# rknightion/iq-to-audio

Measured on AMD Instinct MI355X. Metric: complex IQ MS/s end-to-end (ingest->48 kHz audio), higher is better.
Workload: dtype i8; 1 GPU; BASELINE config 2: synthetic 60 s @ 10 MS/s int16 I/Q, 1 NFM channel, +25 kHz, bw 12.5 kHz, D=104, 6401 taps, chunk 4194304; frames_per_gpu=600000000, parallelism=1 independent capture(s), one per GPU; RCCL gather of 48 kHz audio only, audio_samples_48k=2879996, mix_sign=1, settle_steps=55

## Files before the change

### include/iqa_hotpath.h

```cpp
#ifndef IQA_HOTPATH_H
#define IQA_HOTPATH_H

#include <stdint.h>

#ifdef __cplusplus
extern "C" {
#endif

#define IQA_ABI_VERSION 1
#define IQA_SUMSQ_SLOTS 8

typedef enum {
    IQA_OK = 0,
    IQA_EINVAL = 1,
    IQA_EHIP = 2,
    IQA_ESTATE = 3
} iqa_status;

typedef enum { IQA_FMT_S16 = 0, IQA_FMT_U8 = 1, IQA_FMT_F32 = 2 } iqa_fmt;

typedef enum { IQA_ORDER_IQ = 0, IQA_ORDER_QI = 1, IQA_ORDER_IQ_INV = 2, IQA_ORDER_QI_INV = 3 } iqa_iq_order;

typedef enum { IQA_DEMOD_NFM = 0, IQA_DEMOD_AM = 1, IQA_DEMOD_USB = 2, IQA_DEMOD_LSB = 3 } iqa_demod;

// ... 39 lines not shown
                        const void *raw_dev, int64_t n_frames, int64_t consumed, int64_t m_first, int64_t n_out,
                        void *z_out_dev, void *stream);

typedef struct {
    const void *afrag_dev;
    void *z_out_dev;
    const void *partial_in_dev;
    void *partial_out_dev;
    double unit, c_re, c_im;
    uint64_t rot_step, rot_base;
    float out_scale_re, out_scale_im;
    int32_t q_group, finalize, conj_sum, rotate;
    int32_t raw_partials;
    int32_t reserved;
} iqa_mfma_lane;
int iqa_channelize_mfma_multi(int32_t fmt, int32_t decimation, int32_t k_first, int32_t k_count,
                              int32_t outputs_per_block, const iqa_mfma_lane *lanes, int32_t n_lanes,
                              const void *raw_dev, int64_t n_frames, int64_t consumed, int64_t m_first,
                              int64_t n_out, void *stream);

int iqa_channelize_mfma_pairs(int32_t fmt, int32_t decimation, int32_t k_first, int32_t k_count,
                              int32_t outputs_per_block, const iqa_mfma_lane *lanes, int32_t n_lanes,
                              const void *raw_dev, int64_t n_frames, int64_t consumed, int64_t m_first,
                              int64_t n_out, void *stream);
int32_t iqa_mfma_ring_pairs(int32_t fmt, int32_t decimation, int32_t k_first, int32_t k_count);
int32_t iqa_mfma_ring_lanes(int32_t fmt, int32_t decimation, int32_t k_first, int32_t k_count, int32_t acc32);
int iqa_mfma_combine(const iqa_chan_params *p, const void *const *partials_dev, int32_t n_partials,
                     const double *raw_scale, int64_t m_first, int64_t n_out, void *z_out_dev, void *stream);

int iqa_history_update(int32_t fmt, int32_t ntaps, const void *hist_dev, const void *raw_dev, int64_t n_frames,
                       void *hist_next_dev, void *stream);


int iqa_oscillator_mix(int32_t fmt, int32_t iq_order, const void *in_dev, int64_t n, double phase0, double step,
                       void *out_dev, void *stream);

int iqa_decimate(const void *in_dev, int64_t n, int64_t first, int32_t D, void *out_dev, int64_t n_out,
                 void *stream);

int iqa_mean_power(const void *z_dev, int64_t n, int64_t skip, void *power_dev, void *stream);

int iqa_mean_power_batch(const void *z_dev, int64_t n_each, int32_t parts, int64_t skip, void *power_dev, void *stream);

int iqa_raw_level(int32_t fmt, const void *raw_dev, int64_t n_values, void *mean_square_out, void *stream);


int iqa_quadrature(const void *z_dev, int64_t n, void *prev_dev, void *out_dev, void *stream);

int iqa_envelope(const void *z_dev, int64_t n, void *out_dev, void *stream);

int iqa_real_part(const void *z_dev, int64_t n, void *out_dev, void *stream);

int64_t iqa_scan_workspace_bytes(int64_t n);
int iqa_deemphasis(const void *x_dev, int64_t n, double alpha, void *state_dev, void *y_dev, void *work_dev,
                   void *stream);
int iqa_dc_block(const void *x_dev, int64_t n, double radius, void *state_dev, void *y_dev, void *work_dev,
                 void *stream);
int iqa_agc(const void *x_dev, int64_t n, double target, double decay, const void *reset_starts_dev,
            int64_t n_resets, void *y_dev, void *work_dev, void *stream);

typedef struct {
    int32_t mode;
    int32_t agc_enabled;
    double deemph_alpha;
    double dc_radius;
    double agc_target;
    double agc_decay;
} iqa_demod_params;
int iqa_demodulate(const iqa_demod_params *p, const void *z_dev, int64_t n, void *state_dev,
                   const void *seg_starts_dev, int64_t n_segs, void *peak_dev, void *sumsq_dev, void *audio_out_dev,
                   void *scratch_dev, void *work_dev, void *stream);
int iqa_demodulate_from_reset(const iqa_demod_params *p, const void *z_dev, int64_t n, void *state_dev,
                              const void *seg_starts_dev, int64_t n_segs, void *peak_dev, void *sumsq_dev,
                              void *audio_out_dev, void *scratch_dev, void *work_dev, void *stream);

int iqa_writer_clip(const void *a_dev, int64_t n, void *peak_dev, const void *seg_starts_dev, int64_t n_segs,
                    void *sumsq_dev, void *out_dev, void *stream);

int iqa_resample(const void *x_dev, int64_t n_in, const void *table_dev, int32_t up, int32_t down, int32_t T,
                 int64_t j0, int64_t n_out, void *y_dev, void *pcm16_dev, void *stream);

int iqa_float_to_pcm16(const void *y_dev, int64_t n, void *pcm_dev, void *stream);


#define IQA_WFM_MAX_TAPS 2047
int64_t iqa_wfm_partials(int64_t n);
int iqa_wfm_stereo(int32_t ntaps, const void *taps_dev, float m_scale, const void *theta_dev, int64_t n, const void *hist_dev,
                   void *m_out_dev, void *a_out_dev, void *b_out_dev, void *partials_dev, void *stream);
int iqa_wfm_matrix(const void *a_dev, const void *b_dev, int64_t n, void *left_dev, void *right_dev, void *stream);


#define IQA_RDS_MAX_HALF 2400
#define IQA_RDS_MAX_DECIM 80
int64_t iqa_rds_hist_len(int32_t ntaps, int32_t half_taps);
int64_t iqa_rds_outputs(int64_t pos, int64_t n, int32_t decim);
int64_t iqa_rds_lds_bytes(int32_t ntaps, int32_t half_taps, int32_t decim);
int iqa_rds_baseband(int32_t ntaps, const void *pilot_taps_dev, int32_t half_taps, const void *mf_taps_dev, int32_t decim,
                     float m_scale, double f_mix, double clock_step, const void *theta_dev, int64_t n, int64_t pos,
                     const void *hist_dev, void *y_out_dev, void *q_out_dev, void *stream);
int64_t iqa_rds_clock_chunks(int64_t n);
int iqa_rds_clock(const void *q_dev, int64_t n, int64_t j_first, double clock_step, void *total_dev, void *work_dev,
                  void *phi_out_dev, void *psi_out_dev, void *stream);
int64_t iqa_rds_timing_partials(int64_t n);
int iqa_rds_timing(const void *y_dev, const void *psi_dev, int64_t n, int64_t j0, void *partials_dev, void *out_dev, void *stream);
int iqa_rds_symbols(const void *y_dev, const void *psi_dev, int64_t n, int64_t j0, double tau, int64_t k_first, int64_t nsym,
                    void *sym_out_dev, void *bits_out_dev, void *stream);
int iqa_rds_syndromes(const void *bits_dev, int64_t nbits, void *words_out_dev, void *synd_out_dev, void *stream);


#define IQA_POCSAG_MAX_SPS 384
#define IQA_POCSAG_BAUDS 3
#define IQA_POCSAG_OFFSETS 545
int iqa_pocsag_integrate(const void *theta_dev, int64_t n, const void *hist_dev, int32_t hist_len,
                         const int32_t window[IQA_POCSAG_BAUDS], void *t_out_dev, void *const s_out_dev[IQA_POCSAG_BAUDS],
                         void *stream);
int iqa_pocsag_sync(const void *s_dev, int64_t n, const int32_t offsets[32], int32_t half_bit, void *score_dev,
                    void *list_dev, int64_t capacity, void *count_dev, void *stream);
int iqa_pocsag_codewords(const void *s_dev, int64_t n, const void *list_dev, int64_t nsync, const void *offsets_dev,
                         void *fixed_out_dev, void *raw_out_dev, void *status_out_dev, void *stream);


#define IQA_AFSK_MAX_SPS 400
#define IQA_AFSK_PHASES 8
#define IQA_AFSK_GAINS 3
#define IQA_AFSK_SLOT_BYTES 332
int iqa_afsk_correlate(const void *theta_dev, int64_t n, const void *hist_dev, int32_t window, const void *taps_dev,
                       void *t_out_dev, void *sign_out_dev, void *e1200_out_dev, void *e2200_out_dev, void *stream);
// ... 113 lines not shown
```

### iq-to-audio_amd/_native.py

```python
from __future__ import annotations

import ctypes
import subprocess
from ctypes import c_double, c_float, c_int32, c_int64, c_uint64, c_void_p
from pathlib import Path

import os

PKG_DIR = Path(__file__).resolve().parent
LIB_PATH = Path(os.environ["IQA_LIB"]).resolve() if os.environ.get("IQA_LIB") else PKG_DIR / "libiqa_hotpath.so"
CSRC_DIR = PKG_DIR / "csrc"

IQA_OK, IQA_EINVAL, IQA_EHIP, IQA_ESTATE = 0, 1, 2, 3
FMT_S16, FMT_U8, FMT_F32 = 0, 1, 2
ORDER = {"iq": 0, "qi": 1, "iq_inv": 2, "qi_inv": 3}
ABI_VERSION = 1


class ChanParams(ctypes.Structure):

    _fields_ = [
        ("fmt", c_int32),
        ("ntaps", c_int32),
        ("decimation", c_int32),
# ... 33 lines not shown
    _fields_ = [("method", c_int32), ("auto_floor", c_int32), ("trim", c_int32), ("out_pcm16", c_int32),
                ("margin_db", c_double), ("transient_margin_db", c_double)]


class SquelchSeg(ctypes.Structure):

    _fields_ = [("n", c_int64), ("in_off", c_int64), ("base", c_int64), ("channels", c_int32), ("window", c_int32),
                ("short_window", c_int32), ("long_window", c_int32), ("hold", c_int32), ("fade", c_int32),
                ("lead", c_int32), ("trail", c_int32), ("manual_floor_db", c_double), ("q_index", c_int64 * 6),
                ("q_gamma", c_float * 3), ("reserved", c_int32)]


class SquelchResult(ctypes.Structure):

    _fields_ = [("noise_floor_db", c_double), ("threshold_db", c_double), ("start", c_int64), ("stop", c_int64)]


SQ_TILE = 2048
SQ_METHOD = {"adaptive": 0, "static": 1, "transient": 2}
SQ_STAGE = {"envelope_db": 0, "level": 1, "threshold": 2, "mask": 3, "dilated": 4, "gain": 5}

DEMOD_MODE = {"nfm": 0, "fm": 0, "am": 1, "usb": 2, "ssb": 2, "lsb": 3}

_SIGNATURES = {
    "iqa_abi_version": (ctypes.c_int, []),
    "iqa_last_error": (ctypes.c_char_p, []),
    "iqa_taps_padded_len": (c_int64, [c_int32]),
    "iqa_channelize": (ctypes.c_int, [ctypes.POINTER(ChanParams), c_void_p, c_void_p, c_int64, c_int64, c_void_p,
                                      c_int64, c_int64, c_void_p, c_void_p]),
    "iqa_mfma_afrag_bytes": (c_int64, [c_int32]),
    "iqa_mfma_ring_bytes": (c_int64, [c_int32]),
    "iqa_mfma_ring_lds_bytes": (c_int64, [c_int32, c_int32, c_int32, c_int32, c_int32]),
    "iqa_mfma_ring_mode": (c_int32, [c_int32, c_int32, c_int32, c_int32, c_int32]),
    "iqa_channelize_mfma": (ctypes.c_int, [ctypes.POINTER(ChanParams), ctypes.POINTER(MfmaParams), c_void_p, c_void_p,
                                           c_int64, c_int64, c_int64, c_int64, c_void_p, c_void_p]),
    "iqa_channelize_mfma_multi": (ctypes.c_int, [c_int32, c_int32, c_int32, c_int32, c_int32, ctypes.POINTER(MfmaLane), c_int32,
                                                 c_void_p, c_int64, c_int64, c_int64, c_int64, c_void_p]),
    "iqa_channelize_mfma_pairs": (ctypes.c_int, [c_int32, c_int32, c_int32, c_int32, c_int32, ctypes.POINTER(MfmaLane), c_int32,
                                                 c_void_p, c_int64, c_int64, c_int64, c_int64, c_void_p]),
    "iqa_mfma_ring_pairs": (c_int32, [c_int32, c_int32, c_int32, c_int32]),
    "iqa_mfma_ring_lanes": (c_int32, [c_int32, c_int32, c_int32, c_int32, c_int32]),
    "iqa_mfma_combine": (ctypes.c_int, [ctypes.POINTER(ChanParams), ctypes.POINTER(c_void_p), c_int32, ctypes.POINTER(c_double),
                                        c_int64, c_int64, c_void_p, c_void_p]),
    "iqa_history_update": (ctypes.c_int, [c_int32, c_int32, c_void_p, c_void_p, c_int64, c_void_p, c_void_p]),
    "iqa_oscillator_mix": (ctypes.c_int, [c_int32, c_int32, c_void_p, c_int64, c_double, c_double, c_void_p, c_void_p]),
    "iqa_decimate": (ctypes.c_int, [c_void_p, c_int64, c_int64, c_int32, c_void_p, c_int64, c_void_p]),
    "iqa_mean_power": (ctypes.c_int, [c_void_p, c_int64, c_int64, c_void_p, c_void_p]),
    "iqa_mean_power_batch": (ctypes.c_int, [c_void_p, c_int64, c_int32, c_int64, c_void_p, c_void_p]),
    "iqa_raw_level": (ctypes.c_int, [c_int32, c_void_p, c_int64, c_void_p, c_void_p]),
    "iqa_quadrature": (ctypes.c_int, [c_void_p, c_int64, c_void_p, c_void_p, c_void_p]),
    "iqa_envelope": (ctypes.c_int, [c_void_p, c_int64, c_void_p, c_void_p]),
    "iqa_real_part": (ctypes.c_int, [c_void_p, c_int64, c_void_p, c_void_p]),
    "iqa_scan_workspace_bytes": (c_int64, [c_int64]),
    "iqa_deemphasis": (ctypes.c_int, [c_void_p, c_int64, c_double, c_void_p, c_void_p, c_void_p, c_void_p]),
    "iqa_dc_block": (ctypes.c_int, [c_void_p, c_int64, c_double, c_void_p, c_void_p, c_void_p, c_void_p]),
    "iqa_agc": (ctypes.c_int, [c_void_p, c_int64, c_double, c_double, c_void_p, c_int64, c_void_p, c_void_p, c_void_p]),
    "iqa_demodulate": (ctypes.c_int, [ctypes.POINTER(DemodParams), c_void_p, c_int64, c_void_p, c_void_p, c_int64, c_void_p,
                                      c_void_p, c_void_p, c_void_p, c_void_p, c_void_p]),
    "iqa_demodulate_from_reset": (ctypes.c_int, [ctypes.POINTER(DemodParams), c_void_p, c_int64, c_void_p, c_void_p, c_int64, c_void_p,
                                      c_void_p, c_void_p, c_void_p, c_void_p, c_void_p]),
    "iqa_writer_clip": (ctypes.c_int, [c_void_p, c_int64, c_void_p, c_void_p, c_int64, c_void_p, c_void_p, c_void_p]),
    "iqa_resample": (ctypes.c_int, [c_void_p, c_int64, c_void_p, c_int32, c_int32, c_int32, c_int64, c_int64, c_void_p,
                                    c_void_p, c_void_p]),
    "iqa_float_to_pcm16": (ctypes.c_int, [c_void_p, c_int64, c_void_p, c_void_p]),
    "iqa_trickle_copy": (ctypes.c_int, [c_void_p, c_void_p, c_int64, c_int32, c_void_p]),
    "iqa_f32_to_s16_exact": (ctypes.c_int, [c_void_p, c_int64, c_void_p, c_void_p, c_void_p]),
    "iqa_f32_split_s16": (ctypes.c_int, [c_void_p, c_int64, c_int32, c_void_p, c_void_p, c_void_p, c_void_p]),
    "iqa_psd_frames": (ctypes.c_int, [c_int32, c_int32, c_void_p, c_int64, c_int64, c_int64, c_int32, c_int32, c_int32, c_void_p,
                                      c_double, c_void_p, c_void_p, c_void_p, c_void_p, c_void_p]),
    "iqa_pair_average_rows": (ctypes.c_int, [c_void_p, c_int32, c_int32, c_void_p, c_void_p]),
    "iqa_wfm_partials": (c_int64, [c_int64]),
    "iqa_wfm_stereo": (ctypes.c_int, [c_int32, c_void_p, c_float, c_void_p, c_int64, c_void_p, c_void_p, c_void_p, c_void_p,
                                      c_void_p, c_void_p]),
    "iqa_wfm_matrix": (ctypes.c_int, [c_void_p, c_void_p, c_int64, c_void_p, c_void_p, c_void_p]),
    "iqa_rds_hist_len": (c_int64, [c_int32, c_int32]),
    "iqa_rds_outputs": (c_int64, [c_int64, c_int64, c_int32]),
    "iqa_rds_lds_bytes": (c_int64, [c_int32, c_int32, c_int32]),
    "iqa_rds_baseband": (ctypes.c_int, [c_int32, c_void_p, c_int32, c_void_p, c_int32, c_float, c_double, c_double, c_void_p,
                                        c_int64, c_int64, c_void_p, c_void_p, c_void_p, c_void_p]),
    "iqa_rds_clock_chunks": (c_int64, [c_int64]),
    "iqa_rds_clock": (ctypes.c_int, [c_void_p, c_int64, c_int64, c_double, c_void_p, c_void_p, c_void_p, c_void_p, c_void_p]),
    "iqa_rds_timing_partials": (c_int64, [c_int64]),
    "iqa_rds_timing": (ctypes.c_int, [c_void_p, c_void_p, c_int64, c_int64, c_void_p, c_void_p, c_void_p]),
    "iqa_rds_symbols": (ctypes.c_int, [c_void_p, c_void_p, c_int64, c_int64, c_double, c_int64, c_int64, c_void_p, c_void_p,
                                       c_void_p]),
    "iqa_rds_syndromes": (ctypes.c_int, [c_void_p, c_int64, c_void_p, c_void_p, c_void_p]),
    "iqa_pocsag_integrate": (ctypes.c_int, [c_void_p, c_int64, c_void_p, c_int32, ctypes.POINTER(c_int32), c_void_p,
                                            ctypes.POINTER(c_void_p), c_void_p]),
    "iqa_pocsag_sync": (ctypes.c_int, [c_void_p, c_int64, ctypes.POINTER(c_int32), c_int32, c_void_p, c_void_p, c_int64, c_void_p,
                                       c_void_p]),
    "iqa_pocsag_codewords": (ctypes.c_int, [c_void_p, c_int64, c_void_p, c_int64, c_void_p, c_void_p, c_void_p, c_void_p, c_void_p]),
    "iqa_afsk_correlate": (ctypes.c_int, [c_void_p, c_int64, c_void_p, c_int32, c_void_p, c_void_p, c_void_p, c_void_p, c_void_p, c_void_p]),
    "iqa_afsk_bits": (ctypes.c_int, [c_void_p, c_int64, c_int32, c_double, c_int64, c_void_p, c_void_p]),
    "iqa_afsk_frames": (ctypes.c_int, [c_void_p, c_int64, ctypes.POINTER(c_int64), c_int32, c_double, c_void_p, c_void_p, c_int64,
                                       c_void_p, c_void_p]),
    "iqa_tones_decimate": (ctypes.c_int, [c_void_p, c_int64, c_int64, c_void_p, c_int32, c_void_p, c_void_p, c_void_p]),
    "iqa_tones_bank": (ctypes.c_int, [c_void_p, c_int64, c_int32, c_int32, c_int32, c_void_p, c_void_p, c_void_p, c_void_p]),
    "iqa_tones_decide": (ctypes.c_int, [c_void_p, c_int64, c_void_p, c_void_p, c_int64, c_int32, c_void_p, c_void_p, c_void_p]),
    "iqa_acars_max": (ctypes.c_int, [c_void_p, c_int64, c_void_p, c_void_p]),
    "iqa_acars_detect": (ctypes.c_int, [c_void_p, c_int64, c_int32, c_int32, c_int32, c_void_p, c_int32, c_int32, c_void_p, c_void_p, c_void_p,
                                        c_void_p, c_void_p, c_void_p]),
    "iqa_acars_bits": (ctypes.c_int, [c_void_p, c_int64, c_int32, c_double, c_int64, c_void_p, c_void_p]),
    "iqa_acars_frames": (ctypes.c_int, [c_void_p, c_int64, ctypes.POINTER(c_int64), c_int32, c_double, c_void_p, c_void_p, c_int64,
                                        c_void_p, c_void_p]),
    "iqa_ais_filter": (ctypes.c_int, [c_void_p, c_int64, c_void_p, c_int32, c_void_p, c_void_p, c_void_p, c_void_p]),
    "iqa_ais_symbols": (ctypes.c_int, [c_void_p, c_int64, c_int32, c_double, c_int64, c_void_p, c_void_p]),
    "iqa_ais_frames": (ctypes.c_int, [c_void_p, c_int64, ctypes.POINTER(c_int64), c_int32, c_double, c_void_p, c_void_p, c_int64,
                                      c_void_p, c_void_p]),
    "iqa_adsb_quantise": (ctypes.c_int, [c_void_p, c_int64, c_void_p, c_void_p]),
    "iqa_adsb_search": (ctypes.c_int, [c_void_p, c_int64, c_void_p, ctypes.POINTER(c_int32), c_int32, c_int32, c_void_p, c_void_p, c_void_p,
                                       c_int64, c_void_p, c_void_p]),
    "iqa_squelch_workspace_bytes": (c_int64, [c_int64, c_int32]),
    "iqa_squelch_stage_offset": (c_int64, [c_int64, c_int32, c_int32]),
# ... 85 lines not shown
```

### iq-to-audio_amd/batch.py

```python
from __future__ import annotations

from ctypes import c_int32, c_int64, c_void_p

import numpy as np

from . import _dev as D
from . import _native as N
from . import dsp_plan as P
from .processing import (PRECISION_GUARD, ChannelBank, ChannelDemod, Channelizer, MixSignProbe, Resampler48k, _ChannelKernel,
                         base_precision, immutable_taps, pick_precision, probe_targets, reserve_pinned_scalars)


def reject_wfm(modes) -> None:
    if any((m or "").lower() == "wfm" for m in modes):
        raise ValueError("wfm targets are not supported by the resident batch runners or sharded runs: "
                         "use ProcessingPipeline / MultiChannelPipeline")


def reject_pocsag(pocsag) -> None:
    if pocsag:
        raise ValueError("pocsag=True is not supported by the resident batch runners or sharded runs: "
                         "use ProcessingPipeline / MultiChannelPipeline")


# ... 58 lines not shown
        self.override = mix_sign_override if mix_sign_override in (1, -1) else None
        self.base_precision = precision or base_precision(demod_mode, agc_enabled)
        self.guard = PRECISION_GUARD if precision_guard is None else float(precision_guard)
        self._guarded = bool(self.guard) and self.override is None and (demod_mode or "").lower() in ("nfm", "fm")
        self._spec_sign, self._spec_precision = 1, self.base_precision
        self.redone = dict(sign=0, precision=0)
        self.n_dec = -(-self.n_frames // self.d)
        self.starts = P.chunk_output_starts(self.chunk, self.d, 0, self.n_frames)
        self.rs = Resampler48k(self.fs_ch)
        self.n48 = self.rs.plan.n_out(self.n_dec)
        self.compute = torch.cuda.current_stream()
        self._compute_raw = int(self.compute.cuda_stream)
        self.aux = D.side_stream("aux")
        self.egress = D.side_stream("egress")
        self._ring_done = None
        self.slots = [dict(z=D.empty(self.n_dec, "complex64"), audio=D.empty(self.n_dec, "float32"),
                           pcm_host=torch.empty(self.n48, dtype=torch.int16).pin_memory(), busy=None,
                           dem=ChannelDemod(demod_mode, self.fs_ch, deemph_us=deemph_us, agc_enabled=agc_enabled))
                      for _ in range(self.SLOTS)]
        self._next = 0
        self._graph_streams = [D.side_stream(f"graph{i}") for i in range(int(graph_streams))] if int(graph_streams) > 1 else []
        self._egress_pending = None
        self.egress_workgroups = 8

    def _probe(self, raw_dev, resident: bool):
        if self.override is not None:
            return None
        torch = D.torch_mod()
        warm = raw_dev[: 2 * min(self.chunk, self.n_frames)] if self.fmt != "f32" else raw_dev[: min(self.chunk, self.n_frames)]
        with D.on_stream(self.aux if resident else self.compute, self.compute):
            return MixSignProbe(warm, self.fs, self.f_off, self.taps, self.d, fmt=self.fmt, iq_order=self.iq_order,
                                record_done=False, measure_level=self._guarded)

    def _kernel_for(self, sign: int):
        return lambda name: Channelizer(self.taps, sample_rate=self.fs, freq_offset=self.f_off, mix_sign=sign, decimation=self.d,
                                        fmt=self.fmt, iq_order=self.iq_order, precision=name)._kernel

    def _needed_precision(self, probe, sign: int) -> str:
        if not self._guarded or probe is None:
            return self.base_precision
        memo = self.__dict__.setdefault("_guard_memo", {}).setdefault(sign, {})
        return pick_precision(self._kernel_for(sign), self.base_precision, self.demod_args["mode"], probe.power, probe.wideband_rms,
                              self.guard, memo)

    def _chain(self, raw_dev, slot, sign: int, events=None, halo=None, resident: bool = False, probe=None, precision: str | None = None,
               make_probe=None):
        torch = D.torch_mod()
        chan = Channelizer(self.taps, sample_rate=self.fs, freq_offset=self.f_off, mix_sign=sign, decimation=self.d,
                           fmt=self.fmt, iq_order=self.iq_order, precision=precision or self.base_precision)
        chan.plan_ahead()
        dem = slot["dem"]
        side = self.aux if resident else None
        with D.on_stream(self.aux if resident else self.compute, self.compute):
            dem.reset()
        dem.prepare(self.n_dec, self.starts)
        gate = None
        if events is None:
            gate = torch.cuda.Event()
            gate.record(self.compute)
        prev = self._egress_pending
        chan.process(raw_dev, out_dev=slot["z"], events=events, last_block=True, halo=halo, edge_stream=side)
        if make_probe is not None:
            probe = make_probe()
        if events is None:
            ring_done = torch.cuda.Event()
            ring_done.record(self.compute)
        else:
            gate, ring_done = events[0], events[1]
        self._ring_done = ring_done
        if prev is not None:
            self._flush_egress(gate)
        aux_done = None
        if resident:
            aux_done = torch.cuda.Event()
            aux_done.record(self.aux)
            self.compute.wait_event(aux_done)
        if probe is not None:
            probe._done = [aux_done] if resident else [gate]
        dem.process(slot["z"], self.starts, slot["audio"])
        pcm = self.rs.process(slot["audio"], want="pcm16")
        done = torch.cuda.Event()
        ticket = dict(chan=chan, dem=dem, pcm=pcm, done=done, tail_done=None, kernel=chan._kernel.last_kernel,
                      slot=slot, egress_queued=False, resident=resident, precision=chan.precision, probe=probe)
        self._egress_pending = ticket
        return ticket

    def tail_event(self, ticket: dict):
        if ticket.get("tail_done") is None:
            ev = D.torch_mod().cuda.Event()
            ev.record(self.compute)
            ticket["tail_done"] = ev
        return ticket["tail_done"]

    def _flush_egress(self, gate=None) -> None:
        t = self._egress_pending
        if t is None or t["egress_queued"]:
            return
        torch = D.torch_mod()
        if gate is not None:
            self.egress.wait_event(gate)
        else:
            self.egress.wait_event(self.tail_event(t))
        with D.on_stream(self.egress, self.compute):
            t["pcm"].record_stream(self.egress)
            host = t["slot"]["pcm_host"]
            N.call("iqa_trickle_copy", N.ptr(t["pcm"]), c_void_p(host.data_ptr()), c_int64(host.numel() * host.element_size()),
                   c_int32(self.egress_workgroups if gate is not None else max(self.egress_workgroups, 64)), N.stream_ptr())
# ... 376 lines not shown
```

### iq-to-audio_amd/csrc/demod_fused.hip

```cpp
#include "common.h"

namespace iqa {

constexpr int SC_THREADS = 256;
constexpr int SC_ITEMS = 8;
constexpr int SC_TILE = SC_THREADS * SC_ITEMS;

struct Aff {
    double A, B;
};
__device__ __forceinline__ Aff then(const Aff &l, const Aff &r) { return Aff{r.A * l.A, fma(r.A, l.B, r.B)}; }

__device__ __forceinline__ Aff wave_inclusive(Aff v, int lane)
{
#pragma unroll
    for (int o = 1; o < kWave; o <<= 1) {
        const double la = __shfl_up(v.A, o, kWave);
        const double lb = __shfl_up(v.B, o, kWave);
        if (lane >= o) v = then(Aff{la, lb}, v);
    }
    return v;
}

__device__ __forceinline__ long long lower_bound_ll(const long long *arr, long long n, long long v)
// ... 109 lines not shown
                zz[1] = e1;
            }
        } else {
#pragma unroll
            for (int i = 0; i < SC_ITEMS + 2; ++i) {
                const long long k = base - 2 + i;
                zz[i] = (k >= 0 && k < a.n) ? a.z[k] : make_float2(0.f, 0.f);
            }
        }
        if constexpr (SRC == S_QUAD) {
            if (base == 0) zz[1] = a.fresh ? make_float2(1.f, 0.f) : a.prev[0];
        }
#pragma unroll
        for (int i = 0; i < SC_ITEMS; ++i) u[i] = (base + i < a.n) ? src_value<SRC>(zz[i + 2], zz[i + 1]) : 0.f;
        if constexpr (OP == F_DC) {
            if (base == 0) u_before = a.fresh ? 0.f : static_cast<float>(a.st[0]);
            else u_before = src_value<SRC>(zz[1], zz[0]);
        }
    }
}

template <int OP>
__device__ __forceinline__ Aff fmap(const FusedArgs &a, long long idx, float x, float x_prev, bool maybe_reset)
{
    if constexpr (OP == F_DEEMPH) {
        return Aff{a.p0, a.p1 * static_cast<double>(x)};
    } else if constexpr (OP == F_DC) {
        return Aff{a.p0, static_cast<double>(x - x_prev)};
    } else {
        const float mag = fabsf(x);
        Aff m{1.0, 0.0};
        if (mag > 1e-6f) {
            const float desired = static_cast<float>(a.p0) / mag;
            m = Aff{1.0 - a.p1, a.p1 * static_cast<double>(desired)};
        }
        if (maybe_reset) {
            bool rst = (idx == 0);
            if (!rst && a.segs != nullptr && a.n_segs > 0) {
                const long long lo = lower_bound_ll(a.segs, a.n_segs, idx);
                rst = lo < a.n_segs && a.segs[lo] == idx;
            }
            if (rst) m = Aff{0.0, m.A + m.B};
        }
        return m;
    }
}

__device__ __forceinline__ bool block_has_restart(const FusedArgs &a, long long lo_i, long long hi_i)
{
    if (lo_i == 0) return true;
    if (a.segs == nullptr || a.n_segs <= 0) return false;
    const long long lo = lower_bound_ll(a.segs, a.n_segs, lo_i);
    return lo < a.n_segs && a.segs[lo] < hi_i;
}

template <int OP, int SRC>
__global__ __launch_bounds__(SC_THREADS) void k_fused_reduce(FusedArgs a)
{
    __shared__ Aff s_w[SC_THREADS / kWave];
    const int tid = threadIdx.x, lane = tid & 63, wave = tid >> 6;
    const long long blk0 = static_cast<long long>(blockIdx.x) * SC_TILE;
    const long long base = blk0 + static_cast<long long>(tid) * SC_ITEMS;
    const bool mr = (OP == F_AGC) && block_has_restart(a, blk0, blk0 + SC_TILE);
    float u[SC_ITEMS], ub;
    load_u<OP, SRC>(a, base, u, ub);
    Aff t{1.0, 0.0};
#pragma unroll
    for (int i = 0; i < SC_ITEMS; ++i)
        if (base + i < a.n) t = then(t, fmap<OP>(a, base + i, u[i], i ? u[i - 1] : ub, mr));
    const Aff inc = wave_inclusive(t, lane);
    if (lane == kWave - 1) s_w[wave] = inc;
    __syncthreads();
    if (tid == 0) {
        Aff tot = s_w[0];
#pragma unroll
        for (int w = 1; w < SC_THREADS / kWave; ++w) tot = then(tot, s_w[w]);
        a.agg[blockIdx.x] = tot;
    }
}

constexpr int FC_THREADS = 1024;
template <int OP>
__global__ __launch_bounds__(FC_THREADS) void k_fused_carry(FusedArgs a)
{
    __shared__ Aff s_w[FC_THREADS / kWave];
    const int tid = threadIdx.x, lane = tid & 63, wave = tid >> 6;
    double s0;
    if constexpr (OP == F_DEEMPH) s0 = a.fresh ? 0.0 : a.st[0];
    else if constexpr (OP == F_DC) s0 = a.fresh ? 0.0 : a.st[1];
    else s0 = 1.0;
    const int per = (a.nblocks + FC_THREADS - 1) / FC_THREADS;
    const int b0 = tid * per;
    Aff t{1.0, 0.0};
    for (int i = 0; i < per; ++i)
        if (b0 + i < a.nblocks) t = then(t, a.agg[b0 + i]);
    const Aff inc = wave_inclusive(t, lane);
    if (lane == kWave - 1) s_w[wave] = inc;
    __syncthreads();
    Aff pre{1.0, 0.0};
    for (int w = 0; w < wave; ++w) pre = then(pre, s_w[w]);
    Aff exl{__shfl_up(inc.A, 1, kWave), __shfl_up(inc.B, 1, kWave)};
    if (lane == 0) exl = Aff{1.0, 0.0};
    const Aff ex = then(pre, exl);
    double s = fma(ex.A, s0, ex.B);
    for (int i = 0; i < per; ++i) {
        const int b = b0 + i;
// ... 105 lines not shown
                        run += idx < bnd ? vv : 0.0;
                        run_hi += idx < bnd ? 0.0 : vv;
                    }
                }
            } else {
                vout[i] = v;
            }
        }
    }
    if constexpr (SINK == K_CLIP) {
        if (general && run != 0.0) atomicAdd(&a.sumsq[seg * IQA_SUMSQ_SLOTS + (blockIdx.x & (IQA_SUMSQ_SLOTS - 1))], run);
        pk = wave_max(pk);
        const double wlo = (stats && !general) ? wave_sum(run) : 0.0;
        const double whi = simple ? wave_sum(run_hi) : 0.0;
        if (lane == 0) {
            s_pk[wave] = pk;
            s_sq[wave] = wlo;
            s_sq[4 + wave] = whi;
        }
        __syncthreads();
        if (tid == 0) {
            if (a.peak_bits != nullptr) {
                const unsigned int m = __float_as_uint(fmaxf(fmaxf(s_pk[0], s_pk[1]), fmaxf(s_pk[2], s_pk[3])));
                if (m > __hip_atomic_load(a.peak_bits, __ATOMIC_RELAXED, __HIP_MEMORY_SCOPE_AGENT)) atomicMax(a.peak_bits, m);
            }
            const int sub = blockIdx.x & (IQA_SUMSQ_SLOTS - 1);
            if (stats && !general) atomicAdd(&a.sumsq[seg0 * IQA_SUMSQ_SLOTS + sub], s_sq[0] + s_sq[1] + s_sq[2] + s_sq[3]);
            if (simple) atomicAdd(&a.sumsq[seg1 * IQA_SUMSQ_SLOTS + sub], s_sq[4] + s_sq[5] + s_sq[6] + s_sq[7]);
        }
    }
    if (OP != F_AGC && blockIdx.x == a.nblocks - 1 && tid == 0) {
        if constexpr (SRC == S_QUAD) prev_out[0] = a.z[a.n - 1];
        if constexpr (OP == F_DEEMPH) {
            st_out[0] = a.fin[0];
        } else if constexpr (OP == F_DC) {
            float last;
            if constexpr (SRC == S_F32) last = a.x[a.n - 1];
            else last = src_value<SRC>(a.z[a.n - 1], make_float2(0.f, 0.f));
            st_out[0] = static_cast<double>(last);
            st_out[1] = a.fin[0];
        }
    }
    if (a.y_aligned && base + SC_ITEMS <= a.n) {
        float4 *yp = reinterpret_cast<float4 *>(a.y + base);
        yp[0] = make_float4(vout[0], vout[1], vout[2], vout[3]);
        yp[1] = make_float4(vout[4], vout[5], vout[6], vout[7]);
    } else {
#pragma unroll
        for (int i = 0; i < SC_ITEMS; ++i)
            if (base + i < a.n) a.y[base + i] = vout[i];
    }
}

template <int OP, int SRC, int SINK>
static int launch_fused(FusedArgs a, float2 *prev_out, double *st_out, void *work, hipStream_t s)
{
    a.nblocks = static_cast<int>((a.n + SC_TILE - 1) / SC_TILE);
    char *w = static_cast<char *>(work);
    a.agg = reinterpret_cast<Aff *>(w);
    a.carry = reinterpret_cast<double *>(w + sizeof(Aff) * a.nblocks);
    a.fin = a.carry + a.nblocks;
    hipLaunchKernelGGL((k_fused_reduce<OP, SRC>), dim3(a.nblocks), dim3(SC_THREADS), 0, s, a);
    hipLaunchKernelGGL((k_fused_carry<OP>), dim3(1), dim3(FC_THREADS), 0, s, a);
    FusedArgs b = a;
    b.prev = reinterpret_cast<const float2 *>(a.fin + 1);
    b.st = a.fin + 2;
    b.fresh = 0;
    hipLaunchKernelGGL((k_fused_apply<OP, SRC, SINK>), dim3(a.nblocks), dim3(SC_THREADS), 0, s, b, prev_out, st_out);
    return check_launch("fused demodulator");
}

}

using namespace iqa;

static int demodulate(const iqa_demod_params *p, const void *z_dev, int64_t n, void *state_dev, const void *seg_starts_dev,
                      int64_t n_segs, void *peak_dev, void *sumsq_dev, void *audio_out_dev, void *scratch_dev, void *work_dev,
                      void *stream, int fresh)
{
    if (p == nullptr) return fail_inval("params is NULL");
    if (n < 0 || n_segs < 0) return fail_inval("negative length");
    if (p->mode < IQA_DEMOD_NFM || p->mode > IQA_DEMOD_LSB) return fail_inval("Unsupported demod mode");
    if (n == 0) return IQA_OK;
    if (!z_dev || !state_dev || !audio_out_dev || !work_dev) return fail_inval("NULL device pointer");
    if (n_segs > 0 && !seg_starts_dev) return fail_inval("seg_starts is NULL");
    hipStream_t s = as_stream(stream);
    char *st = static_cast<char *>(state_dev);
    FusedArgs a{};
    a.fresh = fresh;
    a.z = static_cast<const float2 *>(z_dev);
    a.n = n;
    a.segs = static_cast<const long long *>(seg_starts_dev);
    a.n_segs = n_segs;
    a.peak_bits = static_cast<unsigned int *>(peak_dev);
    a.sumsq = static_cast<double *>(sumsq_dev);
    a.y = static_cast<float *>(audio_out_dev);
    a.z_aligned = (reinterpret_cast<uintptr_t>(z_dev) & 15) == 0;
    a.y_aligned = (reinterpret_cast<uintptr_t>(audio_out_dev) & 15) == 0;
    a.prev = reinterpret_cast<const float2 *>(st);
    if (p->mode == IQA_DEMOD_NFM) {
        a.p0 = p->deemph_alpha;
        a.p1 = 1.0 - p->deemph_alpha;
        a.st = reinterpret_cast<const double *>(st + 8);
        return launch_fused<F_DEEMPH, S_QUAD, K_CLIP>(a, reinterpret_cast<float2 *>(st), reinterpret_cast<double *>(st + 8),
                                                      work_dev, s);
    }
    if (!(p->dc_radius > 0.0 && p->dc_radius < 1.0)) return fail_inval("radius must be between 0 and 1");
    a.p0 = static_cast<double>(static_cast<float>(p->dc_radius));
    a.st = reinterpret_cast<const double *>(st + 16);
    double *dc_out = reinterpret_cast<double *>(st + 16);
    if (p->mode == IQA_DEMOD_AM) return launch_fused<F_DC, S_ENV, K_CLIP>(a, nullptr, dc_out, work_dev, s);
    if (!p->agc_enabled) return launch_fused<F_DC, S_REAL, K_CLIP>(a, nullptr, dc_out, work_dev, s);
    if (!scratch_dev) return fail_inval("SSB with AGC needs a float scratch buffer of n elements");
    FusedArgs d = a;
    d.y = static_cast<float *>(scratch_dev);
    d.y_aligned = (reinterpret_cast<uintptr_t>(scratch_dev) & 15) == 0;
    d.peak_bits = nullptr;
    d.sumsq = nullptr;
    int rc = launch_fused<F_DC, S_REAL, K_PLAIN>(d, nullptr, dc_out, work_dev, s);
    if (rc != IQA_OK) return rc;
    FusedArgs g = a;
    g.z = nullptr;
    g.x = static_cast<const float *>(scratch_dev);
    g.p0 = static_cast<double>(static_cast<float>(p->agc_target));
    g.p1 = static_cast<double>(static_cast<float>(p->agc_decay));
    g.st = nullptr;
    return launch_fused<F_AGC, S_F32, K_CLIP>(g, nullptr, nullptr, work_dev, s);
}

extern "C" int iqa_demodulate(const iqa_demod_params *p, const void *z_dev, int64_t n, void *state_dev,
                              const void *seg_starts_dev, int64_t n_segs, void *peak_dev, void *sumsq_dev,
                              void *audio_out_dev, void *scratch_dev, void *work_dev, void *stream)
{
    return demodulate(p, z_dev, n, state_dev, seg_starts_dev, n_segs, peak_dev, sumsq_dev, audio_out_dev, scratch_dev, work_dev, stream, 0);
}

extern "C" int iqa_demodulate_from_reset(const iqa_demod_params *p, const void *z_dev, int64_t n, void *state_dev,
                                         const void *seg_starts_dev, int64_t n_segs, void *peak_dev, void *sumsq_dev,
                                         void *audio_out_dev, void *scratch_dev, void *work_dev, void *stream)
{
    if (n == 0) return fail_inval("iqa_demodulate_from_reset needs samples (an empty block resets nothing)");
    return demodulate(p, z_dev, n, state_dev, seg_starts_dev, n_segs, peak_dev, sumsq_dev, audio_out_dev, scratch_dev, work_dev, stream, 1);
}

extern "C" int64_t iqa_scan_workspace_bytes(int64_t n)
{
    const int64_t nb = (n + SC_TILE - 1) / SC_TILE;
    return nb * (sizeof(Aff) + sizeof(double)) + 64;
}


static FusedArgs stage_args(const void *x_dev, int64_t n, void *y_dev)
{
    FusedArgs a{};
    a.x = static_cast<const float *>(x_dev);
    a.y = static_cast<float *>(y_dev);
    a.n = n;
    a.y_aligned = (reinterpret_cast<uintptr_t>(y_dev) & 15) == 0;
    return a;
}

extern "C" int iqa_deemphasis(const void *x_dev, int64_t n, double alpha, void *state_dev, void *y_dev,
                              void *work_dev, void *stream)
{
    if (n < 0) return fail_inval("negative length");
    if (n == 0) return IQA_OK;
    if (!x_dev || !state_dev || !y_dev || !work_dev) return fail_inval("NULL device pointer");
    FusedArgs a = stage_args(x_dev, n, y_dev);
    a.p0 = alpha;
    a.p1 = 1.0 - alpha;
    a.st = static_cast<const double *>(state_dev);
    return launch_fused<F_DEEMPH, S_F32, K_PLAIN>(a, nullptr, static_cast<double *>(state_dev), work_dev, as_stream(stream));
}

extern "C" int iqa_dc_block(const void *x_dev, int64_t n, double radius, void *state_dev, void *y_dev,
                            void *work_dev, void *stream)
{
    if (n < 0) return fail_inval("negative length");
    if (!(radius > 0.0 && radius < 1.0)) return fail_inval("radius must be between 0 and 1");
    if (n == 0) return IQA_OK;
    if (!x_dev || !state_dev || !y_dev || !work_dev) return fail_inval("NULL device pointer");
    FusedArgs a = stage_args(x_dev, n, y_dev);
    a.p0 = static_cast<double>(static_cast<float>(radius));
    a.st = static_cast<const double *>(state_dev);
    return launch_fused<F_DC, S_F32, K_PLAIN>(a, nullptr, static_cast<double *>(state_dev), work_dev, as_stream(stream));
}

extern "C" int iqa_agc(const void *x_dev, int64_t n, double target, double decay, const void *reset_starts_dev,
                       int64_t n_resets, void *y_dev, void *work_dev, void *stream)
{
    if (n < 0 || n_resets < 0) return fail_inval("negative length");
    if (n == 0) return IQA_OK;
    if (!x_dev || !y_dev || !work_dev) return fail_inval("NULL device pointer");
    FusedArgs a = stage_args(x_dev, n, y_dev);
    a.p0 = static_cast<double>(static_cast<float>(target));
    a.p1 = static_cast<double>(static_cast<float>(decay));
    a.segs = static_cast<const long long *>(reset_starts_dev);
// ... 38 lines not shown
```

### iq-to-audio_amd/processing.py

```python
from __future__ import annotations

import contextlib
import logging
import math
import threading
from ctypes import byref, c_double, c_int32, c_int64
from dataclasses import dataclass
from pathlib import Path

import numpy as np

from . import _dev as D
from . import _native as N
from . import dsp_plan as P
from . import iqio
from .channelizer import (_KERNEL_CACHE, _KERNEL_CACHE_LOCK, _KERNEL_CACHE_MAX, _TAPS_MEMO, ChannelBank,
                          Channelizer, _as_frames, _cached_kernel, _ChannelKernel, _taps_fingerprint, immutable_taps)
from .decoders import create_decoder
from .decoders.adsb import AdsbCore, parse_frames as adsb_parse_frames
from .decoders.ais import AisCore, parse_frames as ais_parse_frames
from .decoders.ax25 import AfskCore, parse_frames as ax25_parse_frames
from .decoders.pocsag import PocsagCore, parse_batches as pocsag_parse_batches
from .decoders.rds import RdsCore, result_from as rds_result_from
from .decoders.acars import AcarsCore, parse_messages as acars_parse_messages
# ... 431 lines not shown
                raise ValueError("pocsag=True needs an nfm target: POCSAG is 2-FSK on a narrowband FM channel (--demod nfm)")
            self.pocsag_core = PocsagCore(P.plan_pocsag(fs_channel))
            self._pocsag_prev = D.from_numpy(np.array([1 + 0j], dtype=np.complex64))
        self.afsk_core = None
        if ax25:
            if self.params.mode != N.DEMOD_MODE["nfm"]:
                raise ValueError("ax25=True needs an nfm target: AX.25 here is Bell-202 AFSK on a narrowband FM channel (--demod nfm)")
            self.afsk_core = AfskCore(P.plan_afsk(fs_channel))
            self._afsk_prev = D.from_numpy(np.array([1 + 0j], dtype=np.complex64))
        self.tones_core = None
        if tones:
            if self.params.mode != N.DEMOD_MODE["nfm"]:
                raise ValueError("tones=True needs an nfm target: CTCSS and DTMF ride on a narrowband FM voice channel (--demod nfm)")
            self.tones_core = TonesCore(P.plan_tones(fs_channel))
            self._tones_prev = D.from_numpy(np.array([1 + 0j], dtype=np.complex64))
        self.acars_core = None
        if acars:
            if self.params.mode != N.DEMOD_MODE["am"]:
                raise ValueError("acars=True needs an am target: ACARS is audio MSK on an AM airband carrier (--demod am)")
            self.acars_core = AcarsCore(P.plan_acars(fs_channel))
        self.ais_core = None
        if ais:
            if self.params.mode != N.DEMOD_MODE["nfm"]:
                raise ValueError("ais=True needs an nfm target: AIS is 9600 bit/s GMSK on a narrowband FM channel (--demod nfm)")
            self.ais_core = AisCore(P.plan_ais(fs_channel))
            self._ais_prev = D.from_numpy(np.array([1 + 0j], dtype=np.complex64))
        self.adsb_core = None
        if adsb:
            if self.params.mode != N.DEMOD_MODE["am"]:
                raise ValueError("adsb=True needs an am target: Mode S squitters are pulses on a 1090 MHz AM channel (--demod am)")
            self.adsb_core = AdsbCore(P.plan_adsb(fs_channel))
        self._needs_scratch = self.params.mode in (N.DEMOD_MODE["usb"], N.DEMOD_MODE["lsb"]) and bool(self.params.agc_enabled)
        self.chunk_sumsq: list = []
        self._blk = None
        self._starts_key = None
        self._fresh = False
        self._from_reset = False
        self._alloc_block(0)

    _STATE0 = np.array([1.0, 0, 0, 0, 0, 0, 0, 0], dtype=np.float32)

    def _alloc_block(self, n_chunks: int) -> None:
        torch = D.torch_mod()
        img = np.zeros(64 + n_chunks * 64, dtype=np.uint8)
        img[:32] = self._STATE0.view(np.uint8)
        self._img, self._img_host = img, None
        self._blk = D.from_numpy(img)
        self._n_chunks = n_chunks
        self.state_dev = self._blk[:32].view(torch.float32)
        self.peak_dev = self._blk[32:36].view(torch.float32)
        self._sumsq = self._blk[64:].view(torch.float64)
        self._fresh = True

    def reset(self, force: bool = False) -> None:
        self.chunk_sumsq = []
        if self.pocsag_core is not None:
            self.pocsag_core.reset()
            self._pocsag_prev = D.from_numpy(np.array([1 + 0j], dtype=np.complex64))
        if self.afsk_core is not None:
            self.afsk_core.reset()
            self._afsk_prev = D.from_numpy(np.array([1 + 0j], dtype=np.complex64))
        if self.tones_core is not None:
            self.tones_core.reset()
            self._tones_prev = D.from_numpy(np.array([1 + 0j], dtype=np.complex64))
        if self.acars_core is not None:
            self.acars_core.reset()
        if self.adsb_core is not None:
            self.adsb_core.reset()
        if self.ais_core is not None:
            self.ais_core.reset()
            self._ais_prev = D.from_numpy(np.array([1 + 0j], dtype=np.complex64))
        if self._fresh and not force:
            return
        self._from_reset = True
        self._fresh = True

    def prepare(self, n: int, chunk_starts: np.ndarray):
        starts64 = np.ascontiguousarray(chunk_starts, dtype=np.int64)
        key = (n, len(starts64), hash(starts64.tobytes()))
        if key != self._starts_key:
            self._starts_dev = D.from_numpy(starts64)
            self._work = D.empty(int(N.lib().iqa_scan_workspace_bytes(n)), "uint8")
            self._scratch = D.empty(n, "float32") if self._needs_scratch else None
            self._starts_key = key
        if self._fresh and not self.chunk_sumsq:
            if len(starts64) != self._n_chunks:
                self._alloc_block(len(starts64))
            sumsq = self._sumsq
        else:
            sumsq = D.zeros(len(starts64) * 8, "float64")
        self._prepared = (n, len(starts64), self._starts_dev, sumsq, self._work, self._scratch)

    def process(self, z_dev, chunk_starts: np.ndarray, out_dev):
        n = int(z_dev.numel())
        if n == 0:
            return
        prep = getattr(self, "_prepared", None)
        if prep is None or prep[0] != n or prep[1] != len(chunk_starts):
            self.prepare(n, chunk_starts)
        _, _, starts_dev, sumsq, work, scratch = self._prepared
        self._prepared = None
        self._fresh = False
        entry = "iqa_demodulate_from_reset" if self._from_reset else "iqa_demodulate"
        self._from_reset = False
        N.call(entry, byref(self.params), N.ptr(z_dev), c_int64(n), N.ptr(self.state_dev), N.ptr(starts_dev),
               c_int64(len(chunk_starts)), N.ptr(self.peak_dev), N.ptr(sumsq), N.ptr(out_dev), N.ptr(scratch), N.ptr(work),
               N.stream_ptr())
        counts = np.diff(np.append(chunk_starts, n))
        self.chunk_sumsq.append((sumsq, counts))
        if self.pocsag_core is not None:
            theta = D.empty(n, "float32")
            N.call("iqa_quadrature", N.ptr(z_dev), c_int64(n), N.ptr(self._pocsag_prev), N.ptr(theta), N.stream_ptr())
            self.pocsag_core.process(theta)
        if self.afsk_core is not None:
            theta = D.empty(n, "float32")
            N.call("iqa_quadrature", N.ptr(z_dev), c_int64(n), N.ptr(self._afsk_prev), N.ptr(theta), N.stream_ptr())
            self.afsk_core.process(theta)
        if self.tones_core is not None:
            theta = D.empty(n, "float32")
            N.call("iqa_quadrature", N.ptr(z_dev), c_int64(n), N.ptr(self._tones_prev), N.ptr(theta), N.stream_ptr())
            self.tones_core.process(theta)
        if self.acars_core is not None:
            env = D.empty(n, "float32")
            N.call("iqa_envelope", N.ptr(z_dev), c_int64(n), N.ptr(env), N.stream_ptr())
            self.acars_core.process(env)
# ... 789 lines not shown
```

Measured before the change: 939,100 MS/s.

## Use windowed overlap scan for de-emphasis and clear demod state ahead on aux stream

For NFM de-emphasis the linear recurrence is now computed by a single-pass windowed kernel. Each block recomputes a warm-up window long enough for alpha^window to decay below 2^-64, so no cross-block aggregate or lookback pass is needed. This replaces the multi-pass scan with workspace and fuses the clip, peak and sum-of-squares sink. It also adds a device-side reset kernel so that resident batches clear state, peak and sumsq on the auxiliary stream ahead of time. The cost is redundant recomputation of the overlap window, and the result depends on the exponential-decay truncation.

After: 950,300 MS/s, median of 6. +1.2%, better.

```diff
diff --git a/include/iqa_hotpath.h b/include/iqa_hotpath.h
--- a/include/iqa_hotpath.h
+++ b/include/iqa_hotpath.h
@@ -115,6 +115,7 @@
 int iqa_real_part(const void *z_dev, int64_t n, void *out_dev, void *stream);
 
 int64_t iqa_scan_workspace_bytes(int64_t n);
+int iqa_scan_window(double alpha, int64_t *window, int64_t *span);
 int iqa_deemphasis(const void *x_dev, int64_t n, double alpha, void *state_dev, void *y_dev, void *work_dev,
                    void *stream);
 int iqa_dc_block(const void *x_dev, int64_t n, double radius, void *state_dev, void *y_dev, void *work_dev,
@@ -136,6 +137,8 @@
 int iqa_demodulate_from_reset(const iqa_demod_params *p, const void *z_dev, int64_t n, void *state_dev,
                               const void *seg_starts_dev, int64_t n_segs, void *peak_dev, void *sumsq_dev,
                               void *audio_out_dev, void *scratch_dev, void *work_dev, void *stream);
+
+int iqa_demod_reset(void *state_dev, void *peak_dev, void *sumsq_dev, int64_t n_sums, void *stream);
 
 int iqa_writer_clip(const void *a_dev, int64_t n, void *peak_dev, const void *seg_starts_dev, int64_t n_segs,
                     void *sumsq_dev, void *out_dev, void *stream);
diff --git a/iq-to-audio_amd/_native.py b/iq-to-audio_amd/_native.py
--- a/iq-to-audio_amd/_native.py
+++ b/iq-to-audio_amd/_native.py
@@ -109,6 +109,7 @@
     "iqa_envelope": (ctypes.c_int, [c_void_p, c_int64, c_void_p, c_void_p]),
     "iqa_real_part": (ctypes.c_int, [c_void_p, c_int64, c_void_p, c_void_p]),
     "iqa_scan_workspace_bytes": (c_int64, [c_int64]),
+    "iqa_scan_window": (ctypes.c_int, [c_double, ctypes.POINTER(c_int64), ctypes.POINTER(c_int64)]),
     "iqa_deemphasis": (ctypes.c_int, [c_void_p, c_int64, c_double, c_void_p, c_void_p, c_void_p, c_void_p]),
     "iqa_dc_block": (ctypes.c_int, [c_void_p, c_int64, c_double, c_void_p, c_void_p, c_void_p, c_void_p]),
     "iqa_agc": (ctypes.c_int, [c_void_p, c_int64, c_double, c_double, c_void_p, c_int64, c_void_p, c_void_p, c_void_p]),
@@ -116,6 +117,7 @@
                                       c_void_p, c_void_p, c_void_p, c_void_p, c_void_p]),
     "iqa_demodulate_from_reset": (ctypes.c_int, [ctypes.POINTER(DemodParams), c_void_p, c_int64, c_void_p, c_void_p, c_int64, c_void_p,
                                       c_void_p, c_void_p, c_void_p, c_void_p, c_void_p]),
+    "iqa_demod_reset": (ctypes.c_int, [c_void_p, c_void_p, c_void_p, c_int64, c_void_p]),
     "iqa_writer_clip": (ctypes.c_int, [c_void_p, c_int64, c_void_p, c_void_p, c_int64, c_void_p, c_void_p, c_void_p]),
     "iqa_resample": (ctypes.c_int, [c_void_p, c_int64, c_void_p, c_int32, c_int32, c_int32, c_int64, c_int64, c_void_p,
                                     c_void_p, c_void_p]),
diff --git a/iq-to-audio_amd/batch.py b/iq-to-audio_amd/batch.py
--- a/iq-to-audio_amd/batch.py
+++ b/iq-to-audio_amd/batch.py
@@ -134,7 +134,7 @@
         dem = slot["dem"]
         side = self.aux if resident else None
         with D.on_stream(self.aux if resident else self.compute, self.compute):
-            dem.reset()
+            dem.reset(ahead=resident)
         dem.prepare(self.n_dec, self.starts)
         gate = None
         if events is None:
diff --git a/iq-to-audio_amd/csrc/demod_fused.hip b/iq-to-audio_amd/csrc/demod_fused.hip
--- a/iq-to-audio_amd/csrc/demod_fused.hip
+++ b/iq-to-audio_amd/csrc/demod_fused.hip
@@ -185,6 +185,131 @@
     if (a.segs == nullptr || a.n_segs <= 0) return false;
     const long long lo = lower_bound_ll(a.segs, a.n_segs, lo_i);
     return lo < a.n_segs && a.segs[lo] < hi_i;
+}
+
+
+template <int THREADS>
+__device__ __forceinline__ void sink_count_segments(const FusedArgs &a, long long seg_first, long long first, long long last,
+                                                    long long *s_seg)
+{
+    const int tid = threadIdx.x, lane = tid & 63;
+    int c0 = (tid < a.n_segs) && seg_first <= first, c1 = (tid < a.n_segs) && seg_first <= last;
+    for (long long kk = tid + THREADS; kk < a.n_segs; kk += THREADS) {
+        const long long st = a.segs[kk];
+        c0 += st <= first;
+        c1 += st <= last;
+    }
+    c0 = static_cast<int>(wave_sum(static_cast<float>(c0)));
+    c1 = static_cast<int>(wave_sum(static_cast<float>(c1)));
+    if (lane == 0 && (c0 | c1)) {
+        atomicAdd(reinterpret_cast<unsigned long long *>(&s_seg[0]), static_cast<unsigned long long>(c0));
+        atomicAdd(reinterpret_cast<unsigned long long *>(&s_seg[1]), static_cast<unsigned long long>(c1));
+    }
+}
+
+struct SinkPlan {
+    bool stats, uniform, simple, general;
+    long long seg0, seg1, bnd;
+    int sub;
+};
+__device__ __forceinline__ SinkPlan sink_plan(const FusedArgs &a, bool stats, const long long *s_seg)
+{
+    SinkPlan p;
+    p.stats = stats;
+    p.seg0 = stats ? s_seg[0] : -1;
+    p.seg1 = stats ? s_seg[1] : -1;
+    p.uniform = stats && (p.seg0 == p.seg1);
+    p.simple = stats && (p.seg1 == p.seg0 + 1);
+    p.general = stats && !p.uniform && !p.simple;
+    p.bnd = a.n;
+    if (p.simple) p.bnd = a.segs[p.seg1];
+    p.sub = blockIdx.x & (IQA_SUMSQ_SLOTS - 1);
+    return p;
+}
+
+struct SinkAcc {
+    float pk = 0.f;
+    double run = 0.0, run_hi = 0.0;
+    long long seg = 0;
+};
+
+template <int SINK>
+__device__ __forceinline__ float sink_item(const FusedArgs &a, const SinkPlan &p, SinkAcc &k, float v, long long idx)
+{
+    if constexpr (SINK != K_CLIP) return v;
+    k.pk = fmaxf(k.pk, fabsf(v));
+    if (p.stats) {
+        const double vv = static_cast<double>(v) * static_cast<double>(v);
+        double run = k.run, run_hi = k.run_hi;
+        long long seg = k.seg;
+        if (p.general) {
+            while (seg + 1 < a.n_segs && a.segs[seg + 1] <= idx) {
+                if (run != 0.0) atomicAdd(&a.sumsq[seg * IQA_SUMSQ_SLOTS + p.sub], run);
+                run = 0.0;
+                ++seg;
+            }
+            run += vv;
+        } else {
+            const bool low = idx < p.bnd;
+            run += low ? vv : 0.0;
+            run_hi += low ? 0.0 : vv;
+        }
+        k.run = run;
+        k.run_hi = run_hi;
+        k.seg = seg;
+    }
+    return fminf(fmaxf(v, -0.99f), 0.99f);
+}
+
+__device__ __forceinline__ void sink_flush_general(const FusedArgs &a, const SinkPlan &p, SinkAcc &k)
+{
+    if (p.general && k.run != 0.0) atomicAdd(&a.sumsq[k.seg * IQA_SUMSQ_SLOTS + p.sub], k.run);
+    if (p.general) k.run = 0.0;
+}
+
+template <int WAVES>
+__device__ __forceinline__ void sink_finish(const FusedArgs &a, const SinkPlan &p, SinkAcc &k, float *s_pk, double *s_sq)
+{
+    const int tid = threadIdx.x, lane = tid & 63, wave = tid >> 6;
+    sink_flush_general(a, p, k);
+    const float pk = wave_max(k.pk);
+    const double wlo = (p.stats && !p.general) ? wave_sum(k.run) : 0.0;
+    const double whi = p.simple ? wave_sum(k.run_hi) : 0.0;
+    if (lane == 0) {
+        s_pk[wave] = pk;
+        s_sq[wave] = wlo;
+        s_sq[WAVES + wave] = whi;
+    }
+    __syncthreads();
+    if (tid == 0) {
+        float m = s_pk[0];
+        double lo = s_sq[0], hi = s_sq[WAVES];
+#pragma unroll
+        for (int w = 1; w < WAVES; ++w) {
+            m = fmaxf(m, s_pk[w]);
+            lo += s_sq[w];
+            hi += s_sq[WAVES + w];
+        }
+        if (a.peak_bits != nullptr) {
+            const unsigned int mb = __float_as_uint(m);
+            if (mb > __hip_atomic_load(a.peak_bits, __ATOMIC_RELAXED, __HIP_MEMORY_SCOPE_AGENT)) atomicMax(a.peak_bits, mb);
+        }
+        if (p.stats && !p.general) atomicAdd(&a.sumsq[p.seg0 * IQA_SUMSQ_SLOTS + p.sub], lo);
+        if (p.simple) atomicAdd(&a.sumsq[p.seg1 * IQA_SUMSQ_SLOTS + p.sub], hi);
+    }
+}
+
+__device__ __forceinline__ void store_items(const FusedArgs &a, long long base, long long lo, long long hi, const float (&vout)[SC_ITEMS])
+{
+    if (a.y_aligned && base >= lo && base + SC_ITEMS <= hi) {
+        float4 *yp = reinterpret_cast<float4 *>(a.y + base);
+        yp[0] = make_float4(vout[0], vout[1], vout[2], vout[3]);
+        yp[1] = make_float4(vout[4], vout[5], vout[6], vout[7]);
+    } else {
+#pragma unroll
+        for (int i = 0; i < SC_ITEMS; ++i)
+            if (base + i >= lo && base + i < hi) a.y[base + i] = vout[i];
+    }
 }
 
 template <int OP, int SRC>
@@ -396,9 +521,142 @@
     }
 }
 
+constexpr int FW_THREADS = 256;
+constexpr int FW_ROUNDS = 4;
+constexpr int FW_WAVES = FW_THREADS / kWave;
+constexpr long long FW_ROUND = static_cast<long long>(FW_THREADS) * SC_ITEMS;
+constexpr long long FW_SPAN = FW_ROUND * FW_ROUNDS;
+
+static int scan_window(double alpha, long long *window)
+{
+    if (!(alpha > 0.0 && alpha < 1.0)) return 1;
+    const double need = 64.0 * log(2.0) / -log(alpha);
+    if (!(need < static_cast<double>(FW_SPAN))) return 1;
+    long long w = 512 * static_cast<long long>(ceil(need / 512.0));
+    if (w < 512) w = 512;
+    while (w > 512 && pow(alpha, static_cast<double>(w - 512)) <= 0x1p-64) w -= 512;
+    while (pow(alpha, static_cast<double>(w)) > 0x1p-64) w += 512;
+    if (2 * w > FW_SPAN) return 1;
+    *window = w;
+    return 0;
+}
+
+template <int SRC>
+__device__ __forceinline__ double windowed_round(const FusedArgs &a, long long base, long long end, bool skip0, Aff *s_w,
+                                                 double &s_run, float (&u)[SC_ITEMS])
+{
+    const int lane = threadIdx.x & 63, wave = threadIdx.x >> 6;
+    float ub;
+    load_u<F_DEEMPH, SRC>(a, base, u, ub);
+    if (skip0 && base == 0) u[0] = 0.f;
+    Aff t{1.0, 0.0};
+#pragma unroll
+    for (int i = 0; i < SC_ITEMS; ++i)
+        if (base + i < end) t = then(t, fmap<F_DEEMPH>(a, base + i, u[i], 0.f, false));
+    const Aff inc = wave_inclusive(t, lane);
+    if (lane == kWave - 1) s_w[wave] = inc;
+    __syncthreads();
+    const double ea = __shfl_up(inc.A, 1, kWave), eb = __shfl_up(inc.B, 1, kWave);
+    Aff ex = (lane == 0) ? Aff{1.0, 0.0} : Aff{ea, eb};
+    Aff acc{1.0, 0.0}, wpre{1.0, 0.0};
+#pragma unroll
+    for (int w = 0; w < FW_WAVES; ++w) {
+        if (w == wave) wpre = acc;
+        acc = then(acc, s_w[w]);
+    }
+    ex = then(wpre, ex);
+    const double s = fma(ex.A, s_run, ex.B);
+    s_run = fma(acc.A, s_run, acc.B);
+    return s;
+}
+
+__global__ __launch_bounds__(FC_THREADS) void k_fused_clear(float *state, unsigned int *peak_bits, double *sumsq, long long n_sums)
+{
+    if (state != nullptr && threadIdx.x < 8) state[threadIdx.x] = threadIdx.x ? 0.f : 1.f;
+    if (threadIdx.x == 0 && peak_bits != nullptr) peak_bits[0] = 0u;
+    if (sumsq != nullptr)
+        for (long long i = threadIdx.x; i < n_sums; i += FC_THREADS) sumsq[i] = 0.0;
+}
+
+template <int SRC, int SINK>
+__global__ __launch_bounds__(FW_THREADS) void k_fused_windowed(FusedArgs a, long long window, float2 *prev_out, double *st_out)
+{
+    __shared__ Aff s_w[2][FW_WAVES];
+    __shared__ float s_pk[FW_WAVES];
+    __shared__ double s_sq[2 * FW_WAVES];
+    __shared__ long long s_seg[2];
+    const int tid = threadIdx.x;
+    const long long own = FW_SPAN - window;
+    const long long own0 = static_cast<long long>(blockIdx.x) * own, own1 = min(own0 + own, a.n);
+    const long long start = blockIdx.x ? own0 - window : 0;
+    const bool skip0 = blockIdx.x != 0;
+    const bool stats = (SINK == K_CLIP) && a.sumsq != nullptr && a.n_segs > 0;
+    double s_run = (blockIdx.x == 0 && !a.fresh) ? a.st[0] : 0.0;
+    long long seg_first = 0;
+    if (stats && tid < a.n_segs) seg_first = a.segs[tid];
+    if (stats && tid < 2) s_seg[tid] = -1;
+    if (stats) {
+        __syncthreads();
+        sink_count_segments<FW_THREADS>(a, seg_first, own0, own1 - 1, s_seg);
+    }
+    SinkPlan plan{};
+    SinkAcc acc;
+    for (int r = 0; r < FW_ROUNDS; ++r) {
+        const long long rbase = start + r * FW_ROUND;
+        if (rbase >= own1) break;
+        const long long base = rbase + static_cast<long long>(tid) * SC_ITEMS;
+        float u[SC_ITEMS];
+        double s = windowed_round<SRC>(a, base, own1, skip0, s_w[r & 1], s_run, u);
+        if (r == 0) plan = sink_plan(a, stats, s_seg);
+        if (base + SC_ITEMS <= own0 || base >= own1) continue;
+        acc.seg = plan.seg0;
+        if (plan.general) acc.seg = lower_bound_ll(a.segs, a.n_segs, max(base, own0) + 1) - 1;
+        float vout[SC_ITEMS];
+#pragma unroll
+        for (int i = 0; i < SC_ITEMS; ++i) {
+            const long long idx = base + i;
+            if (idx < own1) {
+                const Aff mi = fmap<F_DEEMPH>(a, idx, u[i], 0.f, false);
+                s = fma(mi.A, s, mi.B);
+            }
+            vout[i] = 0.f;
+            if (idx >= own0 && idx < own1) vout[i] = sink_item<SINK>(a, plan, acc, static_cast<float>(s), idx);
+        }
+        sink_flush_general(a, plan, acc);
+        store_items(a, base, own0, own1, vout);
+    }
+    if constexpr (SINK == K_CLIP) sink_finish<FW_WAVES>(a, plan, acc, s_pk, s_sq);
+    if (blockIdx.x != 0) return;
+    if (a.nblocks > 1) {
+        const long long t0 = (a.n - window) & ~7LL;
+        s_run = 0.0;
+        __syncthreads();
+        for (int r = 0; t0 + r * FW_ROUND < a.n; ++r) {
+            float u[SC_ITEMS];
+            windowed_round<SRC>(a, t0 + r * FW_ROUND + static_cast<long long>(tid) * SC_ITEMS, a.n, false, s_w[r & 1], s_run, u);
+        }
+    }
+    if (tid == 0) {
+        if constexpr (SRC == S_QUAD) prev_out[0] = a.z[a.n - 1];
+        st_out[0] = s_run;
+    }
+}
+
 template <int OP, int SRC, int SINK>
 static int launch_fused(FusedArgs a, float2 *prev_out, double *st_out, void *work, hipStream_t s)
 {
+    if constexpr (OP == F_DEEMPH) {
+        long long window;
+        if (scan_window(a.p0, &window) == 0) {
+            const long long own = FW_SPAN - window;
+            a.nblocks = static_cast<int>((a.n + own - 1) / own);
+            if (a.fresh && (a.peak_bits != nullptr || a.sumsq != nullptr))
+                hipLaunchKernelGGL(k_fused_clear, dim3(1), dim3(FC_THREADS), 0, s, static_cast<float *>(nullptr), a.peak_bits, a.sumsq,
+                                   a.n_segs * IQA_SUMSQ_SLOTS);
+            hipLaunchKernelGGL((k_fused_windowed<SRC, SINK>), dim3(a.nblocks), dim3(FW_THREADS), 0, s, a, window, prev_out, st_out);
+            return check_launch("windowed demodulator");
+        }
+    }
     a.nblocks = static_cast<int>((a.n + SC_TILE - 1) / SC_TILE);
     char *w = static_cast<char *>(work);
     a.agg = reinterpret_cast<Aff *>(w);
@@ -487,6 +745,25 @@
     return demodulate(p, z_dev, n, state_dev, seg_starts_dev, n_segs, peak_dev, sumsq_dev, audio_out_dev, scratch_dev, work_dev, stream, 1);
 }
 
+extern "C" int iqa_demod_reset(void *state_dev, void *peak_dev, void *sumsq_dev, int64_t n_sums, void *stream)
+{
+    if (n_sums < 0) return fail_inval("negative length");
+    if (!state_dev) return fail_inval("NULL device pointer");
+    if (n_sums > 0 && !sumsq_dev) return fail_inval("sumsq is NULL");
+    hipLaunchKernelGGL(k_fused_clear, dim3(1), dim3(FC_THREADS), 0, as_stream(stream), static_cast<float *>(state_dev),
+                       static_cast<unsigned int *>(peak_dev), static_cast<double *>(sumsq_dev), (long long)n_sums);
+    return check_launch("k_fused_clear");
+}
+
+extern "C" int iqa_scan_window(double alpha, int64_t *window, int64_t *span)
+{
+    long long w = 0;
+    if (scan_window(alpha, &w) != 0) return 1;
+    if (window != nullptr) *window = w;
+    if (span != nullptr) *span = FW_SPAN;
+    return 0;
+}
+
 extern "C" int64_t iqa_scan_workspace_bytes(int64_t n)
 {
     const int64_t nb = (n + SC_TILE - 1) / SC_TILE;
diff --git a/iq-to-audio_amd/processing.py b/iq-to-audio_amd/processing.py
--- a/iq-to-audio_amd/processing.py
+++ b/iq-to-audio_amd/processing.py
@@ -507,7 +507,7 @@
         self._sumsq = self._blk[64:].view(torch.float64)
         self._fresh = True
 
-    def reset(self, force: bool = False) -> None:
+    def reset(self, force: bool = False, ahead: bool = False) -> None:
         self.chunk_sumsq = []
         if self.pocsag_core is not None:
             self.pocsag_core.reset()
@@ -526,6 +526,12 @@
             self.ais_core.reset()
             self._ais_prev = D.from_numpy(np.array([1 + 0j], dtype=np.complex64))
         if self._fresh and not force:
+            return
+        if ahead and self.params.mode == N.DEMOD_MODE["nfm"]:
+            N.call("iqa_demod_reset", N.ptr(self.state_dev), N.ptr(self.peak_dev), N.ptr(self._sumsq), c_int64(self._sumsq.numel()),
+                   N.stream_ptr())
+            self._from_reset = False
+            self._fresh = True
             return
         self._from_reset = True
         self._fresh = True
```
